# NVlabs/EmerNeRF

Hardware: AMD Instinct MI355X
Metric: train rays/sec (8192-ray batch, 128 samples) (higher is better)
Workload: dtype f32

## Files before the change

### emernerf_amd/_lib.py

```python
from __future__ import annotations

import ctypes
import os
from ctypes import c_float, c_int, c_int32, c_int64, c_uint32, c_uint64, c_void_p

_PKG = os.path.dirname(os.path.abspath(__file__))
LIB_PATH = os.path.join(_PKG, "lib", "libemernerf_hip.so")
EMER_MAX_LEVELS = 32

F32, F16 = 0, 1
ACT_NONE, ACT_RELU, ACT_SIGMOID, ACT_TRUNC_EXP = 0, 1, 2, 3
STOT_TYPES = {"uniform": 0, "uniform_lindisp": 1, "lindisp": 2, "sqrt": 3, "log": 4, "uniform_lindisp_0": 5}


class GridDesc(ctypes.Structure):
    _fields_ = [
        ("n_dims", c_uint32), ("n_levels", c_uint32), ("n_features", c_uint32),
        ("log2_hashmap_size", c_uint32), ("base_resolution", c_uint32), ("per_level_scale", c_float),
        ("scale", c_float * EMER_MAX_LEVELS), ("res", c_uint32 * EMER_MAX_LEVELS),
        ("size", c_uint32 * EMER_MAX_LEVELS), ("offset", c_uint32 * EMER_MAX_LEVELS),
        ("hashed", c_uint32 * EMER_MAX_LEVELS), ("n_entries", c_uint32),
    ]


# ... 34 lines not shown
    "emer_scale": [_P, _P, c_float, _P, c_int64, _P],
    "emer_cast_f32_f16": [_P, _P, c_int64, _P],
    "emer_render_weights_fwd": [_P, _P, _P, c_int64, c_int32, _P, _P, _P, _P, _P, _P, _P, _P],
    "emer_render_weights_bwd": [_P, _P, _P, _P, _P, _P, _P, c_int64, c_int32, _P, _P],
    "emer_composite_rgb_fwd": [_P, _P, _P, _P, _P, c_int64, c_int32, _P, _P, _P, _P, _P, _P, _P, _P, _P, _P],
    "emer_composite_rgb_bwd": [_P, _P, _P, _P, _P, _P, _P, _P, _P, _P, _P, _P, c_int64, c_int32, _P, _P, _P, _P],
    "emer_blend_accumulate_fwd": [_P, _P, _P, _P, _P, _P, _P, c_int64, c_int32, _P, _P, _P],
    "emer_blend_accumulate_bwd": [_P, _P, _P, _P, _P, _P, _P, _P, _P, c_int64, c_int32, _P, _P, _P, _P, _P, _P, _P, _P],
    "emer_blend_accumulate_wide_fwd": [_P, _P, _P, _P, _P, _P, c_int64, c_int32, c_int32, _P, _P],
    "emer_blend_accumulate_wide_bwd": [_P, _P, _P, _P, _P, _P, _P, c_int64, c_int32, c_int32, _P, _P, _P, _P, _P, _P, _P],
    "emer_ray_epilogue_fwd": [_P, _P, _P, c_int64, _P, _P, _P, _P, _P],
    "emer_ray_epilogue_bwd": [_P, _P, _P, _P, _P, c_int64, _P, _P, _P],
    "emer_pixel_loss_fwd": [_P, _P, _P, _P, c_int64, c_float, c_float, _P, _P, _P],
    "emer_pixel_loss_bwd": [_P, _P, _P, _P, c_int64, c_float, c_float, _P, _P, _P, _P],
    "emer_reg_losses_fwd": [_P, c_int64, c_float, _P, c_int64, c_float, _P, _P, c_int64, c_float, _P, _P, _P, _P, c_int64, c_float, _P, _P, _P, _P],
    "emer_reg_losses_bwd": [_P, c_int64, c_float, _P, c_int64, c_float, _P, _P, c_int64, c_float, _P, _P, _P, _P, c_int64, c_float, _P, c_float,
                            _P, _P, _P, _P, _P, _P],
    "emer_reg_losses_fwd6": [_P, c_int64, c_float, _P, c_int64, c_float, _P, _P, c_int64, c_float, _P, _P, c_int64, c_float, _P, _P, _P, _P],
    "emer_reg_losses_bwd6": [_P, c_int64, c_float, _P, c_int64, c_float, _P, _P, c_int64, c_float, _P, _P, c_int64, c_float, _P, c_float,
                             _P, _P, _P, _P, _P],
    "emer_lidar_loss": [_P, _P, _P, _P, c_int64, c_int32, c_float, c_float, c_float, c_float, _P, _P, _P, _P, _P, _P],
    "emer_accumulate_fwd": [_P, _P, c_int64, c_int32, c_int32, _P, _P],
    "emer_accumulate_bwd": [_P, _P, _P, c_int64, c_int32, c_int32, _P, _P, _P],
    "emer_linear_fwd": [_P, c_int64, _P, _P, _P, c_int64, c_int64, c_int32, c_int32, c_int, _P, _P],
    "emer_linear_bwd": [_P, c_int64, _P, c_int64, _P, c_int64, _P, _P, _P, c_int64, _P, _P, c_int64, c_int32,
                        c_int32, c_int, _P, _P, _P],
    "emer_mlp_chain": [_P, c_int64, _P],
    "emer_wgrad_segmented": [_P, c_int64, _P, _P, c_int32, _P, _P, c_int64, _P, c_int64, c_int32, c_int32, _P],
    "emer_neck_supported": [c_int32, c_int32, c_int32, c_int32],
    "emer_neck_fwd": [_P, c_int32, c_int32, c_int64, _P, _P, _P, _P, c_int32, _P, _P, _P, _P, _P],
    "emer_neck_bwd": [_P, _P, _P, _P, _P, c_int32, c_int32, c_int64, _P, _P, c_int32, _P, _P, _P, _P, _P],
    "emer_neck_bwd_fused_supported": [c_int32, c_int32, c_int32, c_int32],
    "emer_neck_bwd_fused": [_P, _P, _P, _P, _P, c_int32, c_int32, c_int64, _P, _P, _P, c_int32, _P, _P, _P, c_int64, _P, _P, c_int64, _P, _P],
    "emer_rmlp_supported": [c_int32, c_int32, c_int32, c_int32, c_int32],
    "emer_rmlp_fwd": [_P, c_int64, c_int32, c_int32, c_int32, c_int64, c_int32, _P, _P, _P, _P, _P, _P, c_int32, c_int32, _P, _P, _P, c_int64, _P],
    "emer_rmlp_bwd": [_P, c_int64, _P, _P, c_int32, c_int32, c_int32, c_int64, c_int32, _P, _P, _P, c_int32, _P, _P, _P, c_int64, _P],
    "emer_rmlp_bwd_fused_supported": [c_int32, c_int32, c_int32, c_int32, c_int32],
    "emer_rmlp_bwd_fused": [_P, c_int64, _P, c_int64, _P, c_int64, c_int32, c_int32, c_int32, c_int64, c_int32, _P, _P, _P, _P, _P, c_int32, c_int32,
                            _P, c_int64, _P, _P, c_int64, _P, _P, c_int64, _P, _P, c_int64, _P, _P],
    "emer_rgb_head_fwd": [_P, c_int64, _P, _P, c_int64, c_int64, c_int32, c_int32, _P, _P, _P, _P, _P, _P, _P, _P],
    "emer_field_fwd_supported": [c_int32, c_int32],
    "emer_density_bwd_fused": [_P, _P, _P, c_int32, c_int32, c_int64, _P, _P, _P, _P, _P, _P, c_int64, _P, _P, _P, _P],
    "emer_field_fwd": [_P, c_int32, c_int32, c_int64, c_int32, _P, _P, _P, _P, _P, _P, c_int64, c_int32, _P, _P, _P, _P, _P, _P, _P, _P, _P, _P],
    "emer_rgb_head_bwd": [_P, _P, _P, _P, c_int64, c_int32, c_int32, _P, _P, _P, _P, _P, _P, _P, _P, _P, _P, _P, c_int64, _P, _P],
    "emer_rgb_head_bwd_fused_supported": [c_int32],
    "emer_rgb_head_bwd_recompute": [_P, _P, _P, _P, c_int64, _P, _P, c_int64, c_int64, c_int32, c_int32, _P, _P, _P, _P, _P, _P, _P, _P, c_int64, _P, c_int64,
                                    _P, c_int64, _P, _P],
    "emer_rgb_head_bwd_fused": [_P, _P, _P, _P, _P, c_int64, c_int64, c_int32, c_int32, _P, _P, _P, _P, _P, _P, _P, _P, c_int64, _P, c_int64, _P, c_int64,
                                _P, _P],
    "emer_trunc_exp_fwd": [_P, c_int64, _P, c_int64, _P],
    "emer_trunc_exp_bwd": [_P, _P, _P, c_int64, c_int64, _P],
    "emer_dir_encode": [_P, _P, c_int64, c_int32, c_int, _P],
    "emer_aggregate3_fwd": [_P, c_int64, _P, _P],
    "emer_aggregate3_bwd": [_P, c_int64, _P, _P],
    "emer_aggregate3_density_fwd": [_P, c_int64, c_int32, _P, _P, _P],
    "emer_aggregate3_density_bwd": [_P, _P, _P, c_int64, c_int32, _P, _P],
    "emer_ray_inputs_fwd": [_P, c_int64, _P, c_int64, _P, c_int32, c_int32, c_int32, c_int64, _P, c_int64, _P, c_int64, _P],
    "emer_embed_grad": [_P, c_int64, _P, c_int64, _P, c_int64, c_int64, c_int32, c_int32, _P, _P],
    "emer_ray_pre_fwd": [_P, c_int64, c_int64, c_int32, c_int32, _P, c_int64, _P, _P, c_int64, _P, _P, c_int64, _P],
    "emer_ray_pre_bwd": [_P, _P, c_int64, c_int64, c_int32, c_int32, _P, c_int64, _P, c_int64, _P, c_int64, _P],
    "emer_ray_head_fwd": [_P, c_int64, c_int64, _P, c_int64, _P, _P, c_int32, c_int, _P, _P, _P, _P],
    "emer_ray_head_bwd": [_P, _P, _P, _P, c_int64, _P, c_int64, _P, c_int32, c_int, _P, _P, _P, _P],
    "emer_ray_wgrad": [_P, c_int32, c_int64, _P],
    "emer_ray_jobs": [_P, c_int32, _P],
    "emer_dw_reduce_defer": [_P],
    "emer_sample_uniform": [_P, c_uint64, c_int64, _P, c_int32, c_int32, c_int32, _P, _P, _P, _P],
# ... 123 lines not shown
```

### emernerf_amd/csrc/mlp_fused.hip

```cpp
#include <type_traits>

#include "common.h"
#include "bf16x3.h"

namespace emer {

constexpr int kNThreads = 512;
constexpr int kNeckChunk = 8;

struct WSrc {
    const float *w;
    int64_t sn, sk;
    int32_t n, k;
};

template <int KS> struct Opd { u32x4 h[KS], m[KS], l[KS]; };

template <int KT>
__device__ __forceinline__ void make_opd(const f32x4 (&in)[KT], Opd<(KT + 1) / 2> &o) {
#pragma unroll
    for (int s = 0; s < (KT + 1) / 2; ++s) {
#pragma unroll
        for (int q = 0; q < 4; ++q) {
            const int t = 2 * s + (q >> 1), e = 2 * (q & 1);
            if (t < KT) {
                unsigned h, m, l;
                split3(in[t][e], in[t][e + 1], h, m, l);
                o.h[s][q] = h; o.m[s][q] = m; o.l[s][q] = l;
            } else {
                o.h[s][q] = 0u; o.m[s][q] = 0u; o.l[s][q] = 0u;
            }
        }
// ... 440 lines not shown
__device__ __forceinline__ SwT to_rows(const Opd<KS> &o, int p, const SelE e, float *colsum = nullptr) {
    const u32x4 sel = (p & 1) ? u32x4{0u, 0u, e.a0, e.a1} : u32x4{e.a0, e.a1, 0u, 0u};
    const f32x4 z = {0.0f, 0.0f, 0.0f, 0.0f};
    const f32x4 th = EMER_MF(o.h[p >> 1], sel, z), tm = EMER_MF(o.m[p >> 1], sel, z), tl = EMER_MF(o.l[p >> 1], sel, z);
    SwT t;
    t.h = u32x2{pk_bf16(th[0], th[1]), pk_bf16(th[2], th[3])};
    t.m = u32x2{pk_bf16(tm[0], tm[1]), pk_bf16(tm[2], tm[3])};
    t.l = u32x2{pk_bf16(tl[0], tl[1]), pk_bf16(tl[2], tl[3])};
    if (colsum) *colsum += ((tl[0] + tl[1]) + (tl[2] + tl[3])) + ((tm[0] + tm[1]) + (tm[2] + tm[3])) + ((th[0] + th[1]) + (th[2] + th[3]));
    return t;
}
template <int NA, int NB>
__device__ __forceinline__ void dw_tiles(f32x4 (&acc)[NA][NB], const SwT (&a)[NA], const SwT (&bt)[NB]) {
#define EMER_DW_PASS(X, Y)                                                                   \
    _Pragma("unroll") for (int p = 0; p < NA; ++p)                                           \
        _Pragma("unroll") for (int b = 0; b < NB; ++b) acc[p][b] = EMER_MF16(a[p].X, bt[b].Y, acc[p][b]);
    EMER_DW_PASS(l, h) EMER_DW_PASS(h, l) EMER_DW_PASS(m, m) EMER_DW_PASS(m, h) EMER_DW_PASS(h, m) EMER_DW_PASS(h, h)
#undef EMER_DW_PASS
}

struct SwP { u32x4 h, m, l; };
__device__ __forceinline__ SwP block32(const SwT &ta, const SwT &tb) {
    SwP o;
#define EMER_SWAP(T)                                                                      \
    {                                                                                     \
        const auto r0 = __builtin_amdgcn_permlane16_swap(ta.T[0], tb.T[0], false, false); \
        const auto r1 = __builtin_amdgcn_permlane16_swap(ta.T[1], tb.T[1], false, false); \
        o.T = u32x4{r0[0], r1[0], r0[1], r1[1]};                                          \
    }
    EMER_SWAP(h) EMER_SWAP(m) EMER_SWAP(l)
#undef EMER_SWAP
    return o;
}
template <int NQ>
__device__ __forceinline__ void dw_blocks(f32x16 (&acc)[NQ], const SwP &a, const SwP (&b)[NQ]) {
#define EMER_DWB(X, Y) _Pragma("unroll") for (int q = 0; q < NQ; ++q) acc[q] = EMER_MF32(a.X, b[q].Y, acc[q]);
    EMER_DWB(l, h) EMER_DWB(h, l) EMER_DWB(m, m) EMER_DWB(m, h) EMER_DWB(h, m) EMER_DWB(h, h)
#undef EMER_DWB
}

template <int NP, int NQ>
__device__ __forceinline__ void zero_blocks(f32x16 (&acc)[NP][NQ]) {
#pragma unroll
    for (int P = 0; P < NP; ++P)
#pragma unroll
        for (int Q = 0; Q < NQ; ++Q)
#pragma unroll
            for (int r = 0; r < 16; ++r) acc[P][Q][r] = 0.0f;
}
template <int PITCH, int NP, int NQ>
__device__ __forceinline__ void fold_blocks(float *dst, int w, const f32x16 (&acc)[NP][NQ], int lane) {
    const int j32 = lane & 31, h32 = lane >> 5;
#pragma unroll
    for (int P = 0; P < NP; ++P)
#pragma unroll
        for (int Q = 0; Q < NQ; ++Q)
#pragma unroll
            for (int r = 0; r < 16; ++r) {
                float *q = dst + (32 * P + 8 * (r >> 2) + 4 * h32 + (r & 3)) * PITCH + 32 * Q + j32;
                *q = (w == 0) ? acc[P][Q][r] : *q + acc[P][Q][r];
            }
}
template <int N>
__device__ __forceinline__ void finish_colsums(float (&s)[N]) {
#pragma unroll
    for (int p = 0; p < N; ++p) { s[p] += __shfl_xor(s[p], 16, 64); s[p] += __shfl_xor(s[p], 32, 64); }
// ... 188 lines not shown
    for (int w = 0; w < neckw_threads(KT0, NO) / 64; ++w) {
        if (wave == w) {
#pragma unroll
            for (int P = 0; P < 2 * NO; ++P)
#pragma unroll
                for (int Q = 0; Q < 2; ++Q)
#pragma unroll
                    for (int r = 0; r < 16; ++r) {
                        float *q = r1 + (32 * P + 8 * (r >> 2) + 4 * h32 + (r & 3)) * 64 + 32 * Q + j32;
                        *q = (w == 0) ? bw1[P][Q][r] : *q + bw1[P][Q][r];
                    }
#pragma unroll
            for (int P = 0; P < 2; ++P) {
#pragma unroll
                for (int Q = 0; Q < QB; ++Q)
#pragma unroll
                    for (int r = 0; r < 16; ++r) {
                        if (32 * Q + j32 < K0P) {
                            float *q = r0 + (32 * P + 8 * (r >> 2) + 4 * h32 + (r & 3)) * K0P + 32 * Q + j32;
                            *q = (w == 0) ? bw0[P][Q][r] : *q + bw0[P][Q][r];
                        }
                    }
            }
            if (g == 0) {
                fold_bias(rb1, w, ab1, m);
                fold_bias(rb0, w, ab0, m);
            }
        }
        __syncthreads();
    }
    float *part = a.partials + (int64_t)blockIdx.x * a.stride;
    for (int i = threadIdx.x; i < 64 * NO * 65; i += (int)blockDim.x) part[i] = red[i];
    float *part0 = part + 64 * NO * 65;
    for (int i = threadIdx.x; i < 64 * a.k0; i += (int)blockDim.x) { const int nn = i / a.k0, kk = i - nn * a.k0; part0[i] = r0[nn * K0P + kk]; }
    for (int i = threadIdx.x; i < 64; i += (int)blockDim.x) part0[64 * a.k0 + i] = rb0[i];
}

struct RgbFwdArgs {
    const float *geo; int64_t ld_geo;
    const float *rb0, *rb1; int64_t ld_rb;
    int32_t tiles_per_ray; int64_t n_rays;
    WSrc w0g, w1a, w1g, w2; const float *b2;
    float *a1, *a2;
    float *out;
};

struct RgbFwdLds {
    static constexpr int w0 = 0, w1a = w0 + w3_units(4, 2), w1g = w1a + w3_units(4, 2), w2 = w1g + w3_units(4, 2), units = w2 + w3_units(1, 2);
    static constexpr int n_b2 = 16;
    static constexpr size_t bytes = (size_t)units * 16 + n_b2 * sizeof(float);
};
struct RgbFwdW { W3 w0, w1a, w1g, w2; const float *b2; };
__device__ __forceinline__ void rgb_fwd_stage(u32x4 *base, const RgbFwdArgs &a) {
    stage_w3(base + RgbFwdLds::w0, 4, 2, a.w0g);
    stage_w3(base + RgbFwdLds::w1a, 4, 2, a.w1a);
    stage_w3(base + RgbFwdLds::w1g, 4, 2, a.w1g);
    stage_w3(base + RgbFwdLds::w2, 1, 2, a.w2);
}
__device__ __forceinline__ RgbFwdW rgb_fwd_weights(const u32x4 *base, const float *b2l, int lane) {
    return RgbFwdW{w3_at(base + RgbFwdLds::w0, 4, 2, lane), w3_at(base + RgbFwdLds::w1a, 4, 2, lane), w3_at(base + RgbFwdLds::w1g, 4, 2, lane),
                   w3_at(base + RgbFwdLds::w2, 1, 2, lane), b2l};
}

__device__ __forceinline__ void rgb_fwd_tile(const RgbFwdW &w, const f32x4 (&x)[4], const float *rb0, const float *rb1, float *a1, float *a2, float *outp,
                                             bool keep, bool keep2, unsigned lo64, int j, int m, int g) {
    Opd<2> xo;
// ... 445 lines not shown
    for (int i = threadIdx.x; i < 64 * 64; i += kRWThreads) part[64 * 128 + i] = r0[(i >> 6) * P0 + (i & 63)];
    if ((int)threadIdx.x < 195) {
        float t = 0.0f;
        for (int w = 0; w < kRWThreads / 64; ++w) t += r2[w * 196 + threadIdx.x];
        part[64 * 128 + 64 * 64 + threadIdx.x] = t;
    }
}

__global__ __launch_bounds__(kRWThreads, 1) void rgb_bwdw16_kernel(const RgbBwdWArgs a) {
    extern __shared__ __attribute__((aligned(16))) u32x4 smem[];
    rgb_w_stage_chain(smem, a);
    __syncthreads();
    const RgbWLane L = rgb_w_lane(smem, a);
    const int lane = L.lane, m = L.m, g = L.g, tpr = L.tpr;
    float *stg = reinterpret_cast<float *>(smem + 3 * w3_units(4, 2)) + L.wave * (2048 + 3072);
    using gptr = const __attribute__((address_space(1))) void *;
    using lptr = __attribute__((address_space(3))) void *;
    RgbWAcc st;
    rgb_w_zero(st);
    float yn = 0.0f, dn = 0.0f;
    auto issue = [&](int64_t ray, int j, int buf) {
        const int64_t row0 = (ray * tpr + j) * 16;
        const float *p2 = a.a2 + row0 * 64, *p1 = a.a1 + row0 * 64, *pg = a.geo + row0 * a.ld_geo;
        float *sb = stg + 1024 + 2048 * buf;
#pragma unroll
        for (int p = 0; p < 4; ++p) __builtin_amdgcn_global_load_lds((gptr)(p2 + (L.lo64 + 16u * p)), (lptr)(stg + 256 * p), 16, 0, 0);
#pragma unroll
        for (int p = 0; p < 4; ++p) __builtin_amdgcn_global_load_lds((gptr)(p1 + (L.lo64 + 16u * p)), (lptr)(sb + 256 * p), 16, 0, 0);
#pragma unroll
        for (int p = 0; p < 4; ++p) __builtin_amdgcn_global_load_lds((gptr)(pg + (L.log + 16u * p)), (lptr)(sb + 1024 + 256 * p), 16, 0, 0);
        yn = (a.out + row0 * 3)[L.lo3c];
        dn = (a.dout + row0 * 3)[L.lo3c];
    };
    auto b_tile = [&](const float *tile, int p) -> SwT {
        const float *q = tile + 256 * p + 64 * (m >> 2) + (m & 3) + 16 * g;
        const float v0 = q[0], v1 = q[4], v2 = q[8], v3 = q[12];
        SwT t;
        unsigned h0, m0, l0, h1, m1, l1;
        split3(v0, v1, h0, m0, l0);
        split3(v2, v3, h1, m1, l1);
        t.h = u32x2{h0, h1}; t.m = u32x2{m0, m1}; t.l = u32x2{l0, l1};
        return t;
    };
    int buf = 0;
    auto advance = [&](int64_t ray, int j, int by, int64_t &nr, int &nj) {
        nr = ray; nj = j;
        for (int i = 0; i < by; ++i) {
            int64_t r2 = nr; int j2 = nj + 1;
            if (j2 == tpr) { j2 = 0; r2 = nr + L.n_waves; }
            if (r2 >= a.n_rays) break;
            nr = r2; nj = j2;
        }
    };
    if (L.wave_id < a.n_rays) issue(L.wave_id, 0, 0);
    f32x4 dgp[4];
    float *dgeo_prev = nullptr;
    Frag6 fa, fb;
    ld_frag6(fa, L.w1a, 0, 0);
    for (int64_t ray = L.wave_id; ray < a.n_rays; ray += L.n_waves) {
        float s1c[4] = {0.0f, 0.0f, 0.0f, 0.0f}, s0c[4] = {0.0f, 0.0f, 0.0f, 0.0f};
        for (int j = 0; j < tpr; ++j) {
            float *dgeo = a.dgeo + ((ray * tpr + j) * 16) * 64;
            asm volatile("s_waitcnt vmcnt(0)" ::: "memory");
            rgb_w_store_dgeo(dgeo_prev, dgp, L.lo64);
            f32x4 m2[4];
#pragma unroll
            for (int p = 0; p < 4; ++p) m2[p] = *reinterpret_cast<const f32x4 *>(stg + 256 * p + 4 * lane);
            const float d2 = g < 3 ? dn * yn * (1.0f - yn) : 0.0f;
            const float *sb = stg + 1024 + 2048 * buf;
            asm volatile("s_waitcnt lgkmcnt(0)" ::: "memory");
            {
                int64_t nr; int nj;
                advance(ray, j, 1, nr, nj);
                issue(nr, nj, buf ^ 1);
            }
            buf ^= 1;
            Opd<2> d1o, d0o;
            f32x4 dg[4];
            SwP Bq[4];
            rgb_w_chain(st, L, fa, fb, L.w1a, d2, m2,
                        [&](f32x4 (&m1)[4]) {
#pragma unroll
                            for (int p = 0; p < 4; ++p) m1[p] = *reinterpret_cast<const f32x4 *>(sb + 256 * p + 4 * lane);
                        },
                        [&](int k) {
                            const float *t = sb + 1024 * (k >> 1);
                            Bq[k] = block32(b_tile(t, 2 * (k & 1)), b_tile(t, 2 * (k & 1) + 1));
                        },
                        d1o, d0o, dg);
#pragma unroll
            for (int p = 0; p < 4; ++p) dgp[p] = dg[p];
            dgeo_prev = dgeo;
            EMER_RGBW_SB();
            rgb_w_products(st, L.sel, d1o, d0o, Bq, s1c, s0c);
        }
        rgb_w_store_sums(a, L, ray, s1c, s0c);
    }
    rgb_w_store_dgeo(dgeo_prev, dgp, L.lo64);
    rgb_w_epilogue(st, a, L, smem);
}

struct RgbBwdRArgs : RgbBwdWArgs {
    const float *rb0, *rb1; int64_t ld_rb;
    WSrc w0g, w1a, w1g;
};

template <bool A1_STORED>
__global__ __launch_bounds__(kRWThreads, 1) void rgb_bwdwr_kernel(const RgbBwdRArgs a) {
    extern __shared__ __attribute__((aligned(16))) u32x4 smem[];
    u32x4 *w0fl = smem, *w1afl = w0fl + w3_units(4, 2), *w1gfl = w1afl + w3_units(4, 2), *chain = w1gfl + w3_units(4, 2);
    if (!A1_STORED) stage_w3(w0fl, 4, 2, a.w0g);
    stage_w3(w1afl, 4, 2, a.w1a);
    stage_w3(w1gfl, 4, 2, a.w1g);
    rgb_w_stage_chain(chain, a);
    __syncthreads();
    const RgbWLane L = rgb_w_lane(chain, a);
    const int lane = L.lane, g = L.g, tpr = L.tpr;
    const SelE sel = L.sel;
    const W3 w0f = w3_at(w0fl, 4, 2, lane), w1af = w3_at(w1afl, 4, 2, lane), w1gf = w3_at(w1gfl, 4, 2, lane);
    float *rbl = reinterpret_cast<float *>(chain + 3 * w3_units(4, 2)) + L.wave * 256;
// ... 834 lines not shown
    NeckBwdArgs a;
    a.d0 = d0; a.d1 = d1; a.ddens = ddens; a.dens = dens; a.h1 = h1; a.n = n; a.n_levels = n_levels;
    a.dpre1 = dpre1; a.dcol0 = dcol0; a.dpre0 = dpre0; a.denc = denc_lm;
    a.w0t = WSrc{w0, 1, k0, k0, 64};
    hipStream_t st = as_stream(stream);
    const uint32_t grid = row_chunk_grid(n);
    const int kt1 = n_out == 1 ? 0 : (n_out == 64 || !d1) ? 4 : 8;
    a.w1t = w_view_t(w1, 64, kt1 == 0 ? 1 : 16 * kt1, 64);
    return dispatch_kt0_f<1, 1, 2, 4, 8>(k0, n_feat, [&](auto kt0, auto f) {
        auto go = [&](auto k1) {
            return launch(neck_bwd_kernel<RUNG(kt0), RUNG(f), RUNG(k1)>, grid, kNThreads, NeckBwdLds<RUNG(kt0), RUNG(k1)>::bytes, st, "neck_bwd", a);
        };
        return kt1 == 0 ? go(I<0>{}) : kt1 == 4 ? go(I<4>{}) : go(I<8>{});
    });
}

static inline uint32_t neck_bwdw_grid(int64_t n, int no) { return persistent_grid((n + 15) / 16, neckw_threads(0, no) / 64, 256); }
static constexpr size_t neck_bwdw_lds(int kt0, int no) {
    const size_t w = (size_t)(w3_units(kt0, 2) + w3_units(4, 2 * no) + w3_units(4, (kt0 + 1) / 2)) * 16
                     + (size_t)(64 + (neckw_threads(kt0, no) / 64) * (1024 * no + 384 * kt0)) * sizeof(float);
    const size_t r = (size_t)(64 * no * 65 + 64 * 16 * kt0 + 64) * sizeof(float);
    return w > r ? w : r;
}
static inline int64_t neck_bwdw_stride(int k0, int n_out) { return (int64_t)n_out * 65 + 64 * (int64_t)k0 + 64; }

extern "C" int emer_neck_bwd_fused_supported(int32_t n_levels, int32_t n_feat, int32_t hidden, int32_t n_out) {
    return (emer_neck_supported(n_levels, n_feat, hidden, n_out) && (n_out == 64 || n_out == 128)) ? 1 : 0;
}
static inline bool neck_bwdw_fits(int32_t n_levels, int32_t n_feat, int64_t n) { return n * n_levels * n_feat < (1ll << 30); }
extern "C" int64_t emer_neck_bwd_fused_workspace(int32_t n_levels, int32_t n_feat, int64_t n, int32_t n_out) {
    if (n <= 0 || !emer_neck_bwd_fused_supported(n_levels, n_feat, 64, n_out) || !neck_bwdw_fits(n_levels, n_feat, n)) return 0;
    return (int64_t)neck_bwdw_grid(n, n_out / 64) * neck_bwdw_stride(n_levels * n_feat, n_out);
}
extern "C" int emer_neck_bwd_fused(const float *d0, const float *d1, const float *ddens, const float *dens, const float *enc_lm,
                                   int32_t n_levels, int32_t n_feat, int64_t n, const float *w0, const float *b0, const float *w1, int32_t n_out,
                                   float *denc_lm, float *workspace, float *dw0, int64_t ld_dw0, float *db0, float *dw1, int64_t ld_dw1,
                                   float *db1, void *stream) {
    EMER_REQUIRE(n >= 0, "neck_bwd_fused: negative n");
    if (n == 0) return EMER_OK;
    EMER_REQUIRE(emer_neck_bwd_fused_supported(n_levels, n_feat, 64, n_out), "neck_bwd_fused: unsupported shape L=%d F=%d n_out=%d", n_levels, n_feat, n_out);
    EMER_REQUIRE(neck_bwdw_fits(n_levels, n_feat, n), "neck_bwd_fused: n * L * F must stay below 2^30 (32-bit lane offsets); split the batch or use emer_neck_bwd");
    EMER_REQUIRE(enc_lm && w0 && b0 && w1 && denc_lm && workspace && dw0 && db0 && dw1 && db1, "neck_bwd_fused: null pointer");
    EMER_REQUIRE(!ddens || dens, "neck_bwd_fused: ddens needs the saved density");
    EMER_REQUIRE(!d1 || n_out == 128, "neck_bwd_fused: d1 is the gradient of outputs 64..127 of a 128-output neck");
    const int k0 = n_levels * n_feat;
    EMER_REQUIRE(ld_dw0 >= k0 && ld_dw1 >= 64, "neck_bwd_fused: leading dimension smaller than the row");
    NeckBwdWArgs a;
    a.d0 = d0; a.d1 = d1; a.ddens = ddens; a.dens = dens; a.enc = enc_lm; a.b0 = b0; a.n = n; a.n_levels = n_levels; a.k0 = k0;
    a.w0 = WSrc{w0, k0, 1, 64, k0};
    a.w0t = WSrc{w0, 1, k0, k0, 64};
    a.w1t = WSrc{w1, 1, 64, 64, n_out};
    a.denc = denc_lm; a.partials = workspace; a.stride = neck_bwdw_stride(k0, n_out);
    hipStream_t st = as_stream(stream);
    const int no = n_out / 64;
    const uint32_t grid = neck_bwdw_grid(n, no);
    const int rc = dispatch_kt0_f<1, 1, 2, 4, 8>(k0, n_feat, [&](auto kt0, auto f) {
        auto go = [&](auto nn) {
            return launch(neck_bwdw_kernel<RUNG(kt0), RUNG(f), RUNG(nn)>, grid, neckw_threads(RUNG(kt0), RUNG(nn)), neck_bwdw_lds(RUNG(kt0), RUNG(nn)), st,
                          "neck_bwd_fused", a);
        };
        return no == 1 ? go(I<1>{}) : go(I<2>{});
    });
    if (rc) return rc;
    const DwReduceJob jb[2] = {{0, n_out, 64, dw1, ld_dw1, db1, 0, {0}, {0}, {0}}, {(int64_t)n_out * 65, 64, k0, dw0, ld_dw0, db0, 0, {0}, {0}, {0}}};
    return launch_dw_reduce_multi(workspace, (int32_t)grid, a.stride, 2, jb, st);
}

static inline int64_t dens_bwdw_stride(int k0) { return ((int64_t)64 * k0 + 129 + 3) / 4 * 4; }
extern "C" int64_t emer_density_bwd_fused_workspace(int32_t n_levels, int32_t n_feat, int64_t n) {
    const int k0 = n_levels * n_feat;
    if (n <= 0 || k0 < 1 || k0 > 16 || !emer_neck_supported(n_levels, n_feat, 64, 1)) return 0;
    return (int64_t)row_chunk_grid(n) * dens_bwdw_stride(k0);
}
extern "C" int emer_density_bwd_fused(const float *ddens, const float *dens, const float *enc_lm, int32_t n_levels, int32_t n_feat, int64_t n,
                                      const float *w0, const float *b0, const float *w1, float *denc_lm, float *workspace, float *dw0,
                                      int64_t ld_dw0, float *db0, float *dw1, float *db1, void *stream) {
    EMER_REQUIRE(n >= 0, "density_bwd_fused: negative n");
    if (n == 0) return EMER_OK;
    const int k0 = n_levels * n_feat;
    EMER_REQUIRE(emer_density_bwd_fused_workspace(n_levels, n_feat, n) > 0, "density_bwd_fused: unsupported shape L=%d F=%d (needs L F <= 16)", n_levels, n_feat);
    EMER_REQUIRE(ddens && dens && enc_lm && w0 && w1 && denc_lm && workspace && dw0 && db0 && dw1 && db1 && ld_dw0 >= k0, "density_bwd_fused: bad arguments");
    DensBwdWArgs a;
    a.ddens = ddens; a.dens = dens; a.enc = enc_lm; a.n = n; a.n_levels = n_levels;
    a.w0 = WSrc{w0, k0, 1, 64, k0};
    a.b0 = b0; a.w1 = w1; a.denc = denc_lm; a.partials = workspace; a.stride = dens_bwdw_stride(k0);
    hipStream_t st = as_stream(stream);
    const uint32_t grid = row_chunk_grid(n);
    if (int rc = pick4<1>((k0 + 3) / 4, [&](auto ks4) { return launch(density_bwdw_kernel<RUNG(ks4)>, grid, kNThreads, 0, st, "density_bwd_fused", a, n_feat); }))
        return rc;
// ... 283 lines not shown
```

### emernerf_amd/fused.py

```python
from __future__ import annotations

import contextlib
import functools
import os
import ctypes
from ctypes import c_int32, c_int64, c_void_p
from typing import Optional, Tuple

import torch
from torch import Tensor

from . import _lib, ray_jobs
from ._lib import ACT_NONE, ACT_RELU, ACT_SIGMOID, ACT_TRUNC_EXP

MAX_LAYERS, MAX_SEGS = 6, 3
E15 = 3269017.3724721107


class ChainSeg(ctypes.Structure):
    _fields_ = [("ptr", c_void_p), ("ld", c_int64), ("n_total", c_int64), ("fix_a", c_void_p), ("fix_b", c_void_p),
                ("col", c_int32), ("width", c_int32), ("row_div", c_int32), ("mode", c_int32), ("f", c_int32), ("dst_col", c_int32)]


class ChainLayer(ctypes.Structure):
# ... 109 lines not shown
        if side is not None:
            main = torch.cuda.current_stream(dev)
            side.wait_stream(main)
            for t in [dpre, col0] + [getattr(sg, "_t", None) for sg in segs]:
                if t is not None:
                    t.record_stream(side)
            ctx = torch.cuda.stream(side)
        else:
            ctx = contextlib.nullcontext()
        with ctx:
            n_ws = int(_lib.load().emer_linear_bwd_workspace(M, N, k_total))
            ws = torch.empty((n_ws,), device=dev, dtype=torch.float32)
            need_b = want_bias and out_b is None
            if out_w is None or need_b:
                buf = torch.zeros((N * (k_total if out_w is None else 0) + (N if need_b else 0),), device=dev, dtype=torch.float32)
            dw = buf[:N * k_total].view(N, k_total) if out_w is None else None
            db = (buf[-N:] if need_b else None)
            tw = dw if out_w is None else out_w
            tb = out_b if out_b is not None else db
            assert tw.stride(1) == 1 and tw.dtype == torch.float32 and (tb is None or tb.is_contiguous())
            arr = (ChainSeg * MAX_SEGS)()
            for i, sg in enumerate(segs):
                arr[i] = sg
            _lib.call("emer_wgrad_segmented", _p(dpre), dpre.stride(0), _p(col0), arr, len(segs), _p(ws), _p(tw), tw.stride(0),
                      _p(tb) if want_bias else None, M, N, k_total, _stream(dpre))
    return dw, db


FUSED_WGRAD = True
FUSED_RMLP_WGRAD = os.environ.get("EMER_FUSE_RMLP_WGRAD", "1") != "0"
FUSED_RMLP_WIDE = os.environ.get("EMER_FUSE_RMLP_WIDE", "1") != "0"
FUSED_RGB_WGRAD = os.environ.get("EMER_FUSE_RGB_WGRAD", "1") != "0"
RGB_RECOMPUTE = int(os.environ.get("EMER_RGB_RECOMPUTE", "0"))


def rgb_recompute(n_rays: int, samples_per_ray: int) -> int:
    ok = FUSED_WGRAD and FUSED_RGB_WGRAD and _lib.load().emer_rgb_head_bwd_fused_workspace(n_rays, samples_per_ray) > 0
    return int(RGB_RECOMPUTE) if ok else 0
SIDE_STREAM = None


def join_side_stream() -> None:
    if SIDE_STREAM is not None:
        torch.cuda.current_stream().wait_stream(SIDE_STREAM)


def _sink(p) -> Optional[Tensor]:
    if not _USE_GRAD_SINKS:
        return None
    if not getattr(p, "requires_grad", False):
        return None
    g = getattr(p, "grad", None)
    if g is None or g.dtype != torch.float32 or not g.is_cuda or g.stride(-1) != 1:
        return None
    return g


_USE_GRAD_SINKS = False


@contextlib.contextmanager
def grad_sinks(enabled: bool = True):
    global _USE_GRAD_SINKS
    prev, _USE_GRAD_SINKS = _USE_GRAD_SINKS, bool(enabled)
    try:
        yield
# ... 191 lines not shown
        want_h = any(ctx.needs_input_grad) and not ctx.fused_bwd
        if rider is not None and not want_h and rider.usable(L, F, N, n_out):
            h1, out1 = None, None
            out0, dens = _field_fwd(enc, W0, B0, W1, B1, rider)
        else:
            h1, out0, out1, dens = _neck_fwd(enc, W0, B0, W1, B1, n_out, want_h)
        ctx.save_for_backward(enc, W0, W1, h1, dens, B0)
        ctx.n_out = n_out
        ctx.sinks = tuple(_sink(p) for p in (w0, b0, w1, b1))
        if out1 is None:
            return out0, dens
        return out0, out1, dens

    @staticmethod
    def backward(ctx, *grads):
        enc, W0, W1, h1, dens, B0 = ctx.saved_tensors
        n_out = ctx.n_out
        d0, d1, ddens = (grads[0], None, grads[1]) if n_out == 64 else grads
        if d0 is None and d1 is None and ddens is None:
            return None, None, None, None, None, None
        L, N, F = enc.shape
        dev = enc.device
        d0c = None if d0 is None else _c(d0)
        d1c = None if d1 is None else _c(d1)
        fa = None if ddens is None else _c(ddens)
        denc = torch.empty((L, N, F), device=dev, dtype=torch.float32)
        sw0, sb0, sw1, sb1 = ctx.sinks
        tw1, rw1 = _target(sw1, (n_out, 64), dev)
        tb1, rb1 = _target(sb1, (n_out,), dev)
        tw0, rw0 = _target(sw0, (64, L * F), dev)
        tb0, rb0 = _target(sb0, (64,), dev)
        if ctx.fused_bwd:
            ws = torch.empty((int(_lib.load().emer_neck_bwd_fused_workspace(L, F, N, n_out)),), device=dev, dtype=torch.float32)
            with torch.cuda.device(dev):
                _lib.call("emer_neck_bwd_fused", _p(d0c), _p(d1c), _p(fa), _p(dens), _p(enc), L, F, N, _p(W0), _p(B0), _p(W1), n_out,
                          _p(denc), _p(ws), _p(tw0), tw0.stride(0), _p(tb0), _p(tw1), tw1.stride(0), _p(tb1), _stream(enc))
            return denc, rw0, rb0, rw1, rb1, None
        dpre0 = torch.empty((N, 64), device=dev, dtype=torch.float32)
        col0 = None if fa is None else torch.empty((N,), device=dev, dtype=torch.float32)
        with torch.cuda.device(dev):
            _lib.call("emer_neck_bwd", _p(d0c), _p(d1c), _p(fa), _p(dens), _p(h1), L, F, N, _p(W0), _p(W1), n_out, None, _p(col0),
                      _p(dpre0), _p(denc), _stream(enc))
        if d0c is None:
            d0c = torch.zeros((N, 64), device=dev, dtype=torch.float32)
        wgrad(d0c, [seg(h1, 0, 64)], 64, col0=col0, out_w=tw1[:64], out_b=tb1[:64])
        if n_out == 128 and d1c is not None:
            wgrad(d1c, [seg(h1, 0, 64)], 64, out_w=tw1[64:], out_b=tb1[64:])
        wgrad(dpre0, [seg_lm(enc, 0)], L * F, out_w=tw0, out_b=tb0)
        return denc, rw0, rb0, rw1, rb1, None


def _field_fwd(enc: Tensor, W0, B0, W1, B1, rider: RgbRider):
    L, N, F = enc.shape
    dev = enc.device
    hr = _c(rider.hray)
    RW0, RB0, RW1, RB1, RW2, RB2 = (_c(p) for p in rider.params)
    R, Kh = hr.shape
    geo = torch.empty((N, 64), device=dev, dtype=torch.float32)
    dens = torch.empty((N,), device=dev, dtype=torch.float32)
    rb = ray_jobs.front_rb(rider.hray, rider.params[:4])
    parked = rb is not None
    if not parked:
        rb = torch.empty((R, 128), device=dev, dtype=torch.float32)
    rec = rgb_recompute(R, rider.S) if rider.keep else 0
    a1 = torch.empty((N, 64), device=dev, dtype=torch.float32) if (rider.keep and rec != 1) else None
    a2 = torch.empty((N, 64), device=dev, dtype=torch.float32) if (rider.keep and rec == 0) else None
# ... 657 lines not shown
```

### include/emernerf_hip.h

```cpp
#ifndef EMERNERF_HIP_H
#define EMERNERF_HIP_H

#include <stdint.h>

#ifdef __cplusplus
extern "C" {
#endif

#define EMER_MAX_LEVELS 32

#define EMER_OK 0
#define EMER_E_INVALID (-1)
#define EMER_E_LAUNCH (-2)

#define EMER_F32 0
#define EMER_F16 1

#define EMER_ACT_NONE 0
#define EMER_ACT_RELU 1
#define EMER_ACT_SIGMOID 2
#define EMER_ACT_TRUNC_EXP 3

#define EMER_STOT_UNIFORM 0
#define EMER_STOT_UNIFORM_LINDISP 1
// ... 204 lines not shown
    float *store_exp0;
    int32_t in_col, K, out_col, N, act, accumulate;
    int32_t store_col, store_n, store_mode, store_f;
} emer_chain_layer;

typedef struct emer_chain_desc {
    emer_chain_seg segs[EMER_CHAIN_MAX_SEGS];
    emer_chain_layer layers[EMER_CHAIN_MAX_LAYERS];
    int32_t n_segs, n_layers;
    int32_t buf_cols;
    int32_t _pad;
} emer_chain_desc;

int emer_mlp_chain(const emer_chain_desc *host_desc, int64_t n_rows, void *stream);

int emer_wgrad_segmented(const float *dpre, int64_t ld_dpre, const float *col0,
                         const emer_chain_seg *host_segs, int32_t n_segs, float *workspace, float *dw,
                         int64_t ld_dw, float *dbias, int64_t m, int32_t n, int32_t k, void *stream);

int emer_neck_supported(int32_t n_levels, int32_t n_feat, int32_t hidden, int32_t n_out);
int emer_neck_fwd(const float *enc_lm, int32_t n_levels, int32_t n_feat, int64_t n, const float *w0,
                  const float *b0, const float *w1, const float *b1, int32_t n_out, float *h1,
                  float *out0, float *out1, float *dens, void *stream);
int emer_neck_bwd(const float *d0, const float *d1, const float *ddens, const float *dens, const float *h1,
                  int32_t n_levels, int32_t n_feat, int64_t n, const float *w0, const float *w1,
                  int32_t n_out, float *dpre1, float *dcol0, float *dpre0, float *denc_lm, void *stream);

int emer_neck_bwd_fused_supported(int32_t n_levels, int32_t n_feat, int32_t hidden, int32_t n_out);
int64_t emer_neck_bwd_fused_workspace(int32_t n_levels, int32_t n_feat, int64_t n, int32_t n_out);
int emer_neck_bwd_fused(const float *d0, const float *d1, const float *ddens, const float *dens, const float *enc_lm, int32_t n_levels,
                        int32_t n_feat, int64_t n, const float *w0, const float *b0, const float *w1, int32_t n_out,
                        float *denc_lm, float *workspace, float *dw0, int64_t ld_dw0, float *db0, float *dw1, int64_t ld_dw1,
                        float *db1, void *stream);

int emer_rmlp_supported(int32_t n_layers, int32_t k0, int32_t n_feat, int32_t hidden, int32_t n_out);
int emer_rmlp_fwd(const float *x, int64_t ldx, int32_t n_levels, int32_t n_feat, int32_t k0, int64_t n, int32_t n_layers,
                  const float *w0, const float *b0, const float *w1, const float *b1, const float *w2, const float *b2,
                  int32_t n_out, int32_t final_act, float *h1, float *h2, float *out, int64_t ldo, void *stream);
int emer_rmlp_bwd(const float *dlast, int64_t ldd, const float *h1, const float *h2, int32_t n_levels, int32_t n_feat,
                  int32_t k0, int64_t n, int32_t n_layers, const float *w0, const float *w1, const float *w2, int32_t n_out,
                  float *dpre1, float *dpre0, float *dx, int64_t lddx, void *stream);
int emer_rmlp_bwd_fused_supported(int32_t n_layers, int32_t k0, int32_t n_feat, int32_t hidden, int32_t n_out);
int64_t emer_rmlp_bwd_fused_workspace(int32_t n_layers, int32_t k0, int32_t n_feat, int64_t n, int32_t n_out);
int emer_rmlp_bwd_fused(const float *dout, int64_t ldd, const float *out, int64_t ldo, const float *x, int64_t ldx, int32_t n_levels,
                        int32_t n_feat, int32_t k0, int64_t n, int32_t n_layers, const float *w0, const float *b0, const float *w1,
                        const float *b1, const float *w2, int32_t n_out, int32_t final_act, float *dx, int64_t lddx, float *workspace,
                        float *dw0, int64_t ld_dw0, float *db0, float *dw1, int64_t ld_dw1, float *db1, float *dw2, int64_t ld_dw2,
                        float *db2, void *stream);

int emer_rgb_head_fwd(const float *geo, int64_t ld_geo, const float *rb0, const float *rb1, int64_t ld_rb, int64_t n_rays,
                      int32_t samples_per_ray, int32_t kh, const float *w0, const float *w1,
                      const float *w2, const float *b2, float *a1, float *a2, float *out, void *stream);
int64_t emer_density_bwd_fused_workspace(int32_t n_levels, int32_t n_feat, int64_t n);
int emer_density_bwd_fused(const float *ddens, const float *dens, const float *enc_lm, int32_t n_levels,
                           int32_t n_feat, int64_t n, const float *w0, const float *b0, const float *w1,
                           float *denc_lm, float *workspace, float *dw0, int64_t ld_dw0, float *db0,
                           float *dw1, float *db1, void *stream);

int emer_field_fwd_supported(int32_t n_levels, int32_t n_feat);
int emer_field_fwd(const float *enc_lm, int32_t n_levels, int32_t n_feat, int64_t n_rays, int32_t samples_per_ray,
                   const float *nw0, const float *nb0, const float *nw1, const float *nb1, const float *rb0,
                   const float *rb1, int64_t ld_rb, int32_t kh, const float *w0, const float *w1,
                   const float *w2, const float *b2, float *geo, float *dens, float *a1, float *a2,
                   float *out, void *stream);
int64_t emer_rgb_head_bwd_workspace(int64_t n_rays);
int emer_rgb_head_bwd(const float *dout, const float *out, const float *a1, const float *a2, int64_t n_rays,
// ... 226 lines not shown
```

Measured before the change: 3.556 million.

## Add direct neck backward weight-grad kernel using LDS transpose reads

Adds a new fused neck backward kernel for the 32-feature, single-output-block case. It stages split-bf16 operands in LDS and reads them back transposed with ds_read_tr16 so the weight-gradient MFMA operands need no extra shuffles, and it computes bias column sums from those same reads. It also prefetches the next tile's gradients asynchronously with global_load_lds. A runtime switch, on by default, selects this kernel over the existing one, at the cost of more LDS per wave and extra code.

```diff
diff --git a/emernerf_amd/_lib.py b/emernerf_amd/_lib.py
--- a/emernerf_amd/_lib.py
+++ b/emernerf_amd/_lib.py
@@ -90,6 +90,7 @@
     "emer_neck_bwd": [_P, _P, _P, _P, _P, c_int32, c_int32, c_int64, _P, _P, c_int32, _P, _P, _P, _P, _P],
     "emer_neck_bwd_fused_supported": [c_int32, c_int32, c_int32, c_int32],
     "emer_neck_bwd_fused": [_P, _P, _P, _P, _P, c_int32, c_int32, c_int64, _P, _P, _P, c_int32, _P, _P, _P, c_int64, _P, _P, c_int64, _P, _P],
+    "emer_neck_bwd_path": [c_int32],
     "emer_rmlp_supported": [c_int32, c_int32, c_int32, c_int32, c_int32],
     "emer_rmlp_fwd": [_P, c_int64, c_int32, c_int32, c_int32, c_int64, c_int32, _P, _P, _P, _P, _P, _P, c_int32, c_int32, _P, _P, _P, c_int64, _P],
     "emer_rmlp_bwd": [_P, c_int64, _P, _P, c_int32, c_int32, c_int32, c_int64, c_int32, _P, _P, _P, c_int32, _P, _P, _P, c_int64, _P],
diff --git a/emernerf_amd/csrc/mlp_fused.hip b/emernerf_amd/csrc/mlp_fused.hip
--- a/emernerf_amd/csrc/mlp_fused.hip
+++ b/emernerf_amd/csrc/mlp_fused.hip
@@ -1,3 +1,4 @@
+#include <atomic>
 #include <type_traits>
 
 #include "common.h"
@@ -504,6 +505,45 @@
 #undef EMER_SWAP
     return o;
 }
+__device__ __forceinline__ SwT b_tile(const float *tile, int p, int j, int gg) {
+    const float *q = tile + 256 * p + 64 * (j >> 2) + (j & 3) + 16 * gg;
+    const float v0 = q[0], v1 = q[4], v2 = q[8], v3 = q[12];
+    SwT t;
+    unsigned h0, m0, l0, h1, m1, l1;
+    split3(v0, v1, h0, m0, l0);
+    split3(v2, v3, h1, m1, l1);
+    t.h = u32x2{h0, h1}; t.m = u32x2{m0, m1}; t.l = u32x2{l0, l1};
+    return t;
+}
+constexpr int kTrTile = 3 * 128;
+template <int KS>
+__device__ __forceinline__ void tr_store(float *buf, const Opd<KS> &o, int nt, int m, int g) {
+    u32x2 *w = reinterpret_cast<u32x2 *>(buf) + 4 * m + (g ^ (m >> 2));
+#pragma unroll
+    for (int t = 0; t < 2 * KS; ++t)
+        if (t < nt) {
+            const int s = t >> 1, e = 2 * (t & 1);
+            w[(3 * t + 0) * 64] = u32x2{o.h[s][e], o.h[s][e + 1]};
+            w[(3 * t + 1) * 64] = u32x2{o.m[s][e], o.m[s][e + 1]};
+            w[(3 * t + 2) * 64] = u32x2{o.l[s][e], o.l[s][e + 1]};
+        }
+}
+__device__ __forceinline__ SwT tr_tile(const float *buf, int t, int j, int gg, float *colsum = nullptr) {
+    using v4s = __attribute__((ext_vector_type(4))) short;
+    using ltr = __attribute__((address_space(3))) v4s *;
+    const u32x2 *r = reinterpret_cast<const u32x2 *>(buf) + 16 * gg + 4 * (j >> 2) + ((j & 3) ^ gg);
+    SwT o;
+    o.h = __builtin_bit_cast(u32x2, __builtin_amdgcn_ds_read_tr16_b64_v4i16((ltr)(r + (3 * t + 0) * 64)));
+    o.m = __builtin_bit_cast(u32x2, __builtin_amdgcn_ds_read_tr16_b64_v4i16((ltr)(r + (3 * t + 1) * 64)));
+    o.l = __builtin_bit_cast(u32x2, __builtin_amdgcn_ds_read_tr16_b64_v4i16((ltr)(r + (3 * t + 2) * 64)));
+    if (colsum) {
+        auto lo = [](unsigned u) { return __uint_as_float(u << 16); };
+        auto hi = [](unsigned u) { return __uint_as_float(u & 0xffff0000u); };
+        *colsum += ((lo(o.l[0]) + hi(o.l[0])) + (lo(o.l[1]) + hi(o.l[1]))) + ((lo(o.m[0]) + hi(o.m[0])) + (lo(o.m[1]) + hi(o.m[1])))
+                   + ((lo(o.h[0]) + hi(o.h[0])) + (lo(o.h[1]) + hi(o.h[1])));
+    }
+    return o;
+}
 template <int NQ>
 __device__ __forceinline__ void dw_blocks(f32x16 (&acc)[NQ], const SwP &a, const SwP (&b)[NQ]) {
 #define EMER_DWB(X, Y) _Pragma("unroll") for (int q = 0; q < NQ; ++q) acc[q] = EMER_MF32(a.X, b[q].Y, acc[q]);
@@ -758,6 +798,169 @@
     float *part = a.partials + (int64_t)blockIdx.x * a.stride;
     for (int i = threadIdx.x; i < 64 * NO * 65; i += (int)blockDim.x) part[i] = red[i];
     float *part0 = part + 64 * NO * 65;
+    for (int i = threadIdx.x; i < 64 * a.k0; i += (int)blockDim.x) { const int nn = i / a.k0, kk = i - nn * a.k0; part0[i] = r0[nn * K0P + kk]; }
+    for (int i = threadIdx.x; i < 64; i += (int)blockDim.x) part0[64 * a.k0 + i] = rb0[i];
+}
+
+constexpr int kNeckDirectWave = 1024 + 4 * kTrTile + 2 * kTrTile;
+constexpr size_t neck_bwdw_direct_lds(int kt0) {
+    return (size_t)(w3_units(kt0, 2) + w3_units(4, 2) + w3_units(4, (kt0 + 1) / 2)) * 16 + (size_t)(64 + 8 * kNeckDirectWave) * sizeof(float);
+}
+template <int KT0, int F>
+__global__ __launch_bounds__(512, 2) void neck_bwdw_direct_kernel(const NeckBwdWArgs a) {
+    static_assert(KT0 == 2, "32-feature blocks of the encoding without a half-empty one, and the LDS budget");
+    static_assert(neck_bwdw_direct_lds(KT0) <= 160 * 1024, "LDS of neck_bwdw_direct_kernel");
+    static_assert((64 * 65 + 64 * 16 * KT0 + 64) * sizeof(float) <= (size_t)(w3_units(KT0, 2) + w3_units(4, 2) + w3_units(4, KT0 / 2)) * 16,
+                  "the final reduction takes the place of the weights, in front of the staging");
+    extern __shared__ __attribute__((aligned(16))) u32x4 smem[];
+    constexpr int K0P = 16 * KT0, KS0 = KT0 / 2, QB = KT0 / 2;
+    u32x4 *w0l = smem, *w1l = w0l + w3_units(KT0, 2), *w0fl = w1l + w3_units(4, 2);
+    float *b0l = reinterpret_cast<float *>(w0fl + w3_units(4, KS0));
+    stage_w3(w0l, KT0, 2, a.w0t);
+    stage_w3(w1l, 4, 2, a.w1t);
+    stage_w3(w0fl, 4, KS0, a.w0);
+    stage_b(b0l, 64, a.b0, 64);
+    __syncthreads();
+    const int wave = __builtin_amdgcn_readfirstlane(threadIdx.x >> 6), lane = threadIdx.x & 63, m = lane & 15, g = lane >> 4;
+    const W3 w0p = w3_at(w0l, KT0, 2, lane), w1p = w3_at(w1l, 4, 2, lane), w0fp = w3_at(w0fl, 4, KS0, lane);
+    f32x16 bw1[2][2], bw0[2][QB];
+    float ab1[4], ab0[4];
+    zero_blocks(bw1);
+    zero_blocks(bw0);
+#pragma unroll
+    for (int p = 0; p < 4; ++p) { ab1[p] = 0.0f; ab0[p] = 0.0f; }
+    const int64_t n_tiles = (a.n + 15) >> 4, n_waves = (int64_t)gridDim.x * (blockDim.x >> 6);
+    const int64_t per_wave = (n_tiles + n_waves - 1) / n_waves;
+    const int64_t t_begin = ((int64_t)blockIdx.x * (blockDim.x >> 6) + wave) * per_wave;
+    const int64_t t_end = t_begin + per_wave < n_tiles ? t_begin + per_wave : n_tiles;
+    float *stg = b0l + 64 + wave * kNeckDirectWave;
+    float *trb = stg + 1024, *trx = trb + 4 * kTrTile;
+    using gptr = const __attribute__((address_space(1))) void *;
+    using lptr = __attribute__((address_space(3))) void *;
+    f32x4 xn[KT0];
+    float ddn = 0.0f, den = 0.0f;
+    auto issue = [&](int64_t tile) {
+        const int64_t row0 = tile * 16;
+        const unsigned mrow = row0 + m < a.n ? (unsigned)m : (unsigned)(a.n - 1 - row0);
+        const unsigned o64 = mrow * 64u + 4u * g;
+        if (a.d0) {
+            const float *d0 = a.d0 + row0 * 64;
+#pragma unroll
+            for (int p = 0; p < 4; ++p) __builtin_amdgcn_global_load_lds((gptr)(d0 + (o64 + 16u * p)), (lptr)(stg + 256 * p), 16, 0, 0);
+        }
+        ld_lm_t<KT0, F>(a.enc + row0 * F, (unsigned)a.n, a.n_levels, mrow, g, xn);
+        ddn = a.ddens ? (a.ddens + row0)[mrow] : 0.0f;
+        den = a.ddens ? (a.dens + row0)[mrow] : 0.0f;
+    };
+    if (t_begin < t_end) issue(t_begin);
+    f32x4 dep[KT0];
+    int64_t tile_prev = -1;
+    for (int64_t tile = t_begin; tile < t_end; ++tile) {
+        f32x4 d[4], x[KT0];
+        asm volatile("s_waitcnt vmcnt(0)" ::: "memory");
+        if (tile_prev >= 0) st_lm_t<KT0, F>(a.denc + tile_prev * 16 * F, (unsigned)a.n, a.n_levels, (unsigned)m, tile_prev * 16 + m < a.n, g, dep);
+#pragma unroll
+        for (int p = 0; p < 4; ++p) d[p] = a.d0 ? *reinterpret_cast<const f32x4 *>(stg + 256 * p + 4 * lane) : f32x4{0.0f, 0.0f, 0.0f, 0.0f};
+#pragma unroll
+        for (int b = 0; b < KT0; ++b) x[b] = xn[b];
+        const float dd = ddn, de0 = den;
+        asm volatile("s_waitcnt lgkmcnt(0)" ::: "memory");
+        issue(tile + 1 < t_end ? tile + 1 : tile);
+        const int64_t row = tile * 16 + m;
+        const bool ok = row < a.n;
+        const float fix = ok ? trunc_exp_bwd(dd, de0) : 0.0f;
+        SwP hq[2];
+        unsigned relu_bits = 0u;
+        {
+#pragma unroll
+            for (int b = 0; b < KT0; ++b)
+#pragma unroll
+                for (int i = 0; i < 4; ++i) x[b][i] = ok ? x[b][i] : 0.0f;
+            Opd<KS0> xo;
+            make_opd<KT0>(x, xo);
+            tr_store<KS0>(trx, xo, KT0, m, g);
+            f32x4 h[4];
+            init_bias<4>(b0l, g, h);
+            tgemm<KS0, 4, false>(w0fp, xo, h);
+#pragma unroll
+            for (int p = 0; p < 4; ++p)
+#pragma unroll
+                for (int i = 0; i < 4; ++i) {
+                    h[p][i] = (ok && h[p][i] > 0.0f) ? h[p][i] : 0.0f;
+                    relu_bits |= (h[p][i] > 0.0f ? 1u : 0u) << (4 * p + i);
+                }
+            Opd<2> ho;
+            make_opd<4>(h, ho);
+            tr_store<2>(trb, ho, 4, m, g);
+        }
+        f32x4 da[4];
+        zero<4>(da);
+        {
+#pragma unroll
+            for (int p = 0; p < 4; ++p)
+#pragma unroll
+                for (int i = 0; i < 4; ++i) d[p][i] = ok ? d[p][i] : 0.0f;
+            if (g == 0) d[0][0] += fix;
+            Opd<2> dop;
+            make_opd<4>(d, dop);
+#pragma unroll
+            for (int q = 0; q < 2; ++q) hq[q] = block32(tr_tile(trb, 2 * q, m, g), tr_tile(trb, 2 * q + 1, m, g));
+            tr_store<2>(trb, dop, 4, m, g);
+            tgemm<2, 4, false>(w1p, dop, da);
+#pragma unroll
+            for (int P = 0; P < 2; ++P) {
+                const SwT t0 = tr_tile(trb, 2 * P, m, g, &ab1[2 * P]), t1 = tr_tile(trb, 2 * P + 1, m, g, &ab1[2 * P + 1]);
+                dw_blocks<2>(bw1[P], block32(t0, t1), hq);
+                __builtin_amdgcn_sched_barrier(0);
+            }
+        }
+#pragma unroll
+        for (int p = 0; p < 4; ++p)
+#pragma unroll
+            for (int i = 0; i < 4; ++i) da[p][i] = ((relu_bits >> (4 * p + i)) & 1u) ? da[p][i] : 0.0f;
+        Opd<2> dao;
+        make_opd<4>(da, dao);
+        tr_store<2>(trb, dao, 4, m, g);
+        f32x4 de[KT0];
+        zero<KT0>(de);
+        tgemm<2, KT0, false>(w0p, dao, de);
+#pragma unroll
+        for (int b = 0; b < KT0; ++b) dep[b] = de[b];
+        tile_prev = tile;
+        {
+            SwP xq[QB];
+#pragma unroll
+            for (int q = 0; q < QB; ++q) xq[q] = block32(tr_tile(trx, 2 * q, m, g), tr_tile(trx, 2 * q + 1, m, g));
+#pragma unroll
+            for (int P = 0; P < 2; ++P) {
+                const SwT t0 = tr_tile(trb, 2 * P, m, g, &ab0[2 * P]), t1 = tr_tile(trb, 2 * P + 1, m, g, &ab0[2 * P + 1]);
+                dw_blocks<QB>(bw0[P], block32(t0, t1), xq);
+                __builtin_amdgcn_sched_barrier(0);
+            }
+        }
+    }
+    if (tile_prev >= 0) st_lm_t<KT0, F>(a.denc + tile_prev * 16 * F, (unsigned)a.n, a.n_levels, (unsigned)m, tile_prev * 16 + m < a.n, g, dep);
+    asm volatile("s_waitcnt vmcnt(0)" ::: "memory");
+    __syncthreads();
+    float *red = reinterpret_cast<float *>(smem);
+    float *r1 = red, *rb1 = r1 + 64 * 64, *r0 = rb1 + 64, *rb0 = r0 + 64 * K0P;
+    finish_colsums(ab1);
+    finish_colsums(ab0);
+#pragma nounroll
+    for (int w = 0; w < 8; ++w) {
+        if (wave == w) {
+            fold_blocks<64>(r1, w, bw1, lane);
+            fold_blocks<K0P>(r0, w, bw0, lane);
+            if (g == 0) {
+                fold_bias(rb1, w, ab1, m);
+                fold_bias(rb0, w, ab0, m);
+            }
+        }
+        __syncthreads();
+    }
+    float *part = a.partials + (int64_t)blockIdx.x * a.stride;
+    for (int i = threadIdx.x; i < 64 * 65; i += (int)blockDim.x) part[i] = red[i];
+    float *part0 = part + 64 * 65;
     for (int i = threadIdx.x; i < 64 * a.k0; i += (int)blockDim.x) { const int nn = i / a.k0, kk = i - nn * a.k0; part0[i] = r0[nn * K0P + kk]; }
     for (int i = threadIdx.x; i < 64; i += (int)blockDim.x) part0[64 * a.k0 + i] = rb0[i];
 }
@@ -1269,16 +1472,6 @@
         yn = (a.out + row0 * 3)[L.lo3c];
         dn = (a.dout + row0 * 3)[L.lo3c];
     };
-    auto b_tile = [&](const float *tile, int p) -> SwT {
-        const float *q = tile + 256 * p + 64 * (m >> 2) + (m & 3) + 16 * g;
-        const float v0 = q[0], v1 = q[4], v2 = q[8], v3 = q[12];
-        SwT t;
-        unsigned h0, m0, l0, h1, m1, l1;
-        split3(v0, v1, h0, m0, l0);
-        split3(v2, v3, h1, m1, l1);
-        t.h = u32x2{h0, h1}; t.m = u32x2{m0, m1}; t.l = u32x2{l0, l1};
-        return t;
-    };
     int buf = 0;
     auto advance = [&](int64_t ray, int j, int by, int64_t &nr, int &nj) {
         nr = ray; nj = j;
@@ -1322,7 +1515,7 @@
                         },
                         [&](int k) {
                             const float *t = sb + 1024 * (k >> 1);
-                            Bq[k] = block32(b_tile(t, 2 * (k & 1)), b_tile(t, 2 * (k & 1) + 1));
+                            Bq[k] = block32(b_tile(t, 2 * (k & 1), m, g), b_tile(t, 2 * (k & 1) + 1, m, g));
                         },
                         d1o, d0o, dg);
 #pragma unroll
@@ -2223,6 +2416,12 @@
     if (n <= 0 || !emer_neck_bwd_fused_supported(n_levels, n_feat, 64, n_out) || !neck_bwdw_fits(n_levels, n_feat, n)) return 0;
     return (int64_t)neck_bwdw_grid(n, n_out / 64) * neck_bwdw_stride(n_levels * n_feat, n_out);
 }
+static std::atomic<int> g_neck_bwd_path{1};
+extern "C" int emer_neck_bwd_path(int32_t path) {
+    EMER_REQUIRE(path == 0 || path == 1, "neck_bwd_path: path %d (0: matrix-pipe transposes, 1: LDS reads)", path);
+    g_neck_bwd_path.store(path, std::memory_order_relaxed);
+    return EMER_OK;
+}
 extern "C" int emer_neck_bwd_fused(const float *d0, const float *d1, const float *ddens, const float *dens, const float *enc_lm,
                                    int32_t n_levels, int32_t n_feat, int64_t n, const float *w0, const float *b0, const float *w1, int32_t n_out,
                                    float *denc_lm, float *workspace, float *dw0, int64_t ld_dw0, float *db0, float *dw1, int64_t ld_dw1,
@@ -2245,7 +2444,12 @@
     hipStream_t st = as_stream(stream);
     const int no = n_out / 64;
     const uint32_t grid = neck_bwdw_grid(n, no);
+    const bool direct = g_neck_bwd_path.load(std::memory_order_relaxed) == 1;
     const int rc = dispatch_kt0_f<1, 1, 2, 4, 8>(k0, n_feat, [&](auto kt0, auto f) {
+        if constexpr (RUNG(kt0) == 2 && RUNG(f) != 1) {
+            if (direct && no == 1)
+                return launch(neck_bwdw_direct_kernel<RUNG(kt0), RUNG(f)>, grid, 512, neck_bwdw_direct_lds(RUNG(kt0)), st, "neck_bwd_fused", a);
+        }
         auto go = [&](auto nn) {
             return launch(neck_bwdw_kernel<RUNG(kt0), RUNG(f), RUNG(nn)>, grid, neckw_threads(RUNG(kt0), RUNG(nn)), neck_bwdw_lds(RUNG(kt0), RUNG(nn)), st,
                           "neck_bwd_fused", a);
diff --git a/emernerf_amd/fused.py b/emernerf_amd/fused.py
--- a/emernerf_amd/fused.py
+++ b/emernerf_amd/fused.py
@@ -165,6 +165,8 @@
 FUSED_RMLP_WIDE = os.environ.get("EMER_FUSE_RMLP_WIDE", "1") != "0"
 FUSED_RGB_WGRAD = os.environ.get("EMER_FUSE_RGB_WGRAD", "1") != "0"
 RGB_RECOMPUTE = int(os.environ.get("EMER_RGB_RECOMPUTE", "0"))
+NECK_BWD = int(os.environ.get("EMER_NECK_BWD", "1"))
+_neck_bwd_applied = None
 
 
 def rgb_recompute(n_rays: int, samples_per_ray: int) -> int:
@@ -422,6 +424,10 @@
         tb0, rb0 = _target(sb0, (64,), dev)
         if ctx.fused_bwd:
             ws = torch.empty((int(_lib.load().emer_neck_bwd_fused_workspace(L, F, N, n_out)),), device=dev, dtype=torch.float32)
+            global _neck_bwd_applied
+            if _neck_bwd_applied != NECK_BWD:
+                _lib.call("emer_neck_bwd_path", int(NECK_BWD))
+                _neck_bwd_applied = NECK_BWD
             with torch.cuda.device(dev):
                 _lib.call("emer_neck_bwd_fused", _p(d0c), _p(d1c), _p(fa), _p(dens), _p(enc), L, F, N, _p(W0), _p(B0), _p(W1), n_out,
                           _p(denc), _p(ws), _p(tw0), tw0.stride(0), _p(tb0), _p(tw1), tw1.stride(0), _p(tb1), _stream(enc))
diff --git a/include/emernerf_hip.h b/include/emernerf_hip.h
--- a/include/emernerf_hip.h
+++ b/include/emernerf_hip.h
@@ -260,6 +260,7 @@
                         int32_t n_feat, int64_t n, const float *w0, const float *b0, const float *w1, int32_t n_out,
                         float *denc_lm, float *workspace, float *dw0, int64_t ld_dw0, float *db0, float *dw1, int64_t ld_dw1,
                         float *db1, void *stream);
+int emer_neck_bwd_path(int32_t path);
 
 int emer_rmlp_supported(int32_t n_layers, int32_t k0, int32_t n_feat, int32_t hidden, int32_t n_out);
 int emer_rmlp_fwd(const float *x, int64_t ldx, int32_t n_levels, int32_t n_feat, int32_t k0, int64_t n, int32_t n_layers,
```

After: 3.577 million (median of 6 runs). Within noise of the previous version (+0.6%).
